# tensorlink-lab/tensorlink

Measured on NVIDIA H100. Metric: generate tokens/sec, higher is better.
Workload: dtype bf16

## Files before the change

include/tensorlink_b200.h:

```cpp
#ifndef TENSORLINK_B200_H
#define TENSORLINK_B200_H

#include <stddef.h>
#include <stdint.h>

#ifdef __cplusplus
extern "C" {
#endif

#define TL_ABI_VERSION 1

typedef enum {
    TL_OK = 0,
    TL_ERR_INVALID = -1,
    TL_ERR_CUDA = -2,
    TL_ERR_NO_DEVICE = -3,
    TL_ERR_WORKSPACE = -4
} tl_status;

#define TL_EPI_BIAS 1
#define TL_EPI_RESIDUAL 2
#define TL_EPI_SWIGLU 4
#define TL_EPI_OUT_F32 8
#define TL_EPI_ACCUM 16
#define TL_A_MN_MAJOR 32
#define TL_B_MN_MAJOR 64

int tl_abi_version(void);
const char* tl_last_error(void);
int tl_device_info(int* sm_count, int* cc_major, int* cc_minor);

int tl_rmsnorm_fwd(const void* x, const void* w, void* y, float* rstd_out, int rows, int H, float eps, void* stream);

int tl_embed_fwd(const int64_t* ids, const void* table, void* out, int n_tokens, int H, int vocab, void* stream);

int tl_gemm_bf16(const void* A, const void* B, void* C, int M, int N, int K, int lda, int ldb, int ldc,
                 const void* bias, const void* residual, int flags, void* stream);

size_t tl_gemm_splitk_ws(int M, int N);
int tl_gemm_bf16_ws(const void* A, const void* B, void* C, int M, int N, int K, int lda, int ldb, int ldc,
                    const void* bias, const void* residual, int flags, void* workspace, size_t ws_bytes, void* stream);
int tl_gemm_bf16_ws_norm(const void* A, const void* B, void* C, int M, int N, int K, int lda, int ldb, int ldc,
                         const void* bias, const void* residual, int flags, void* workspace, size_t ws_bytes,
                         const void* norm_w, float eps, void* H_out, void* stream);

int tl_gemv_bf16(const void* x, const void* W, void* y, int M, int N, int K, const void* bias,
                 const void* residual, const void* norm_w, float eps, int flags, void* stream);
int tl_gemv_bf16_pf(const void* x, const void* W, void* y, int M, int N, int K, const void* bias,
                    const void* residual, const void* norm_w, float eps, int flags, const void* next_W,
                    size_t next_bytes, void* stream);
#define TL_GEMV_COUNTER_WORDS 4
int tl_gemv_bf16_ctr(const void* x, const void* W, void* y, int M, int N, int K, const void* bias,
                     const void* residual, const void* norm_w, float eps, int flags, unsigned* counter,
                     const void* next_W, size_t next_bytes, void* stream);

#define TL_FP8_BLOCK 128
int tl_gemv_fp8(const void* x, const void* W, const float* scales, void* y, int M, int N, int K, const void* bias,
                const void* residual, const void* norm_w, float eps, int flags, void* stream);
int tl_gemv_fp8_ctr(const void* x, const void* W, const float* scales, void* y, int M, int N, int K, const void* bias,
                    const void* residual, const void* norm_w, float eps, int flags, unsigned* counter,
                    const void* next_W, size_t next_bytes, void* stream);
int tl_dequant_fp8(const void* W, const float* scales, void* out, int N, int K, void* stream);

int tl_rope_table(const float* inv_freq, void* cos_tab, void* sin_tab, int max_pos, int half_dim, void* stream);

int tl_rope_kv_fwd(const void* qkv, void* q_out, void* k_cache, void* v_cache, const int32_t* pos0_dev,
                   const void* cos_tab, const void* sin_tab, const void* q_norm_w, const void* k_norm_w,
                   float eps, int n_tokens, int S, int n_h, int n_kv, int d, int T_max, void* stream);

int tl_attn_prefill_fwd(const void* q, const void* k_cache, const void* v_cache, void* out, float* lse, int B,
// ... 182 lines not shown
```

tensorlink_b200/csrc/gemm.cu:

```cuda
#include <stdlib.h>

#include <mutex>
#include <unordered_map>

#include "gemm_common.cuh"

namespace tl {

constexpr int GEMM_THREADS = 384;

typedef CUresult (*EncodeTiledFn)(CUtensorMap*, CUtensorMapDataType, cuuint32_t, void*, const cuuint64_t*,
                                  const cuuint64_t*, const cuuint32_t*, const cuuint32_t*, CUtensorMapInterleave,
                                  CUtensorMapSwizzle, CUtensorMapL2promotion, CUtensorMapFloatOOBfill);

static EncodeTiledFn get_encode_fn() {
    static EncodeTiledFn fn = nullptr;
    static std::once_flag once;
    std::call_once(once, [] {
        void* p = nullptr;
        cudaDriverEntryPointQueryResult q;
        if (cudaGetDriverEntryPoint("cuTensorMapEncodeTiled", &p, cudaEnableDefault, &q) == cudaSuccess &&
            q == cudaDriverEntryPointSuccess)
            fn = (EncodeTiledFn)p;
        else
// ... 33 lines not shown
        if (it != cache.end()) {
            *out = it->second;
            return TL_OK;
        }
    }
    EncodeTiledFn enc = get_encode_fn();
    TL_REQUIRE(enc != nullptr, TL_ERR_CUDA, "cuTensorMapEncodeTiled not available from the driver");
    TL_REQUIRE(((uintptr_t)ptr & 15) == 0 && (ld * 2) % 16 == 0, TL_ERR_INVALID,
               "GEMM operand must be 16-byte aligned with a 16-byte-multiple row pitch (ptr=%p ld=%llu)", ptr,
               (unsigned long long)ld);
    cuuint64_t dims[2] = {inner, outer};
    cuuint64_t strides[1] = {ld * 2};
    cuuint32_t box[2] = {box_inner, box_outer};
    cuuint32_t estr[2] = {1, 1};
    CUresult r = enc(out, CU_TENSOR_MAP_DATA_TYPE_BFLOAT16, 2, const_cast<void*>(ptr), dims, strides, box, estr,
                     CU_TENSOR_MAP_INTERLEAVE_NONE, CU_TENSOR_MAP_SWIZZLE_128B, CU_TENSOR_MAP_L2_PROMOTION_L2_256B,
                     CU_TENSOR_MAP_FLOAT_OOB_FILL_NONE);
    TL_REQUIRE(r == CUDA_SUCCESS, TL_ERR_CUDA, "cuTensorMapEncodeTiled failed (%d) inner=%llu outer=%llu ld=%llu",
               (int)r, (unsigned long long)inner, (unsigned long long)outer, (unsigned long long)ld);
    std::lock_guard<std::mutex> g(mu);
    if (cache.size() > 4096) cache.clear();
    cache[key] = *out;
    return TL_OK;
}

template <int BN>
struct GemmCfg {
    static constexpr int A_BYTES = BM * BK * 2;
    static constexpr int B_BYTES = BN * BK * 2;
    static constexpr int STAGE_BYTES = A_BYTES + B_BYTES;
    static constexpr int STAGES = (BN == 128) ? 4 : 8;
    static constexpr int ACC_PITCH = BN + 4;
    static constexpr int ACC_BYTES = 64 * ACC_PITCH * 4;
    static constexpr int UNITS = BN >= 64 ? 2 * (BN / 64) : 2;
    static_assert(UNITS <= 4 && UNITS * EPI_STAGE_BYTES <= ACC_BYTES, "epilogue staging must fit in the accumulator tile");
    static constexpr int SMEM_BYTES = STAGES * STAGE_BYTES + 2 * ACC_BYTES + 1024  + 256 ;
};

__device__ __forceinline__ void named_bar_sync(int id, int threads) {
    asm volatile("bar.sync %0, %1;" ::"r"(id), "r"(threads) : "memory");
}

template <int BN, bool A_MN, bool B_MN>
__global__ void __launch_bounds__(GEMM_THREADS, 1)
gemm_bf16_kernel(const __grid_constant__ CUtensorMap tmA, const __grid_constant__ CUtensorMap tmB, void* __restrict__ Cv,
                 int M, int N, int K, int ldc, const bf16* __restrict__ bias, const bf16* __restrict__ residual,
                 int ldr, int flags, int k_splits, int kb_per) {
    using Cfg = GemmCfg<BN>;
    extern __shared__ unsigned char smem_dyn[];
    unsigned char* smem = reinterpret_cast<unsigned char*>((reinterpret_cast<uintptr_t>(smem_dyn) + 1023) & ~(uintptr_t)1023);
    float* acc_tile = reinterpret_cast<float*>(smem + Cfg::STAGES * Cfg::STAGE_BYTES);
    uint64_t* bars = reinterpret_cast<uint64_t*>(smem + Cfg::STAGES * Cfg::STAGE_BYTES + 2 * Cfg::ACC_BYTES);
    uint64_t* full_bar = bars;
    uint64_t* empty_bar = bars + Cfg::STAGES;

    const int wg = threadIdx.x >> 7, warp = threadIdx.x >> 5, lane = threadIdx.x & 31;
    const int tiles_m = (M + BM - 1) / BM, tiles_n = (N + BN - 1) / BN;
    const int mn_tiles = tiles_m * tiles_n;
    const int total_tiles = mn_tiles * k_splits;
    const int num_k = (K + BK - 1) / BK;

    if (threadIdx.x == 0) {
        tma_prefetch_desc(&tmA);
        tma_prefetch_desc(&tmB);
        for (int s = 0; s < Cfg::STAGES; ++s) {
            mbar_init(&full_bar[s], 1);
            mbar_init(&empty_bar[s], 8);
        }
        fence_barrier_init();
    }
    __syncthreads();

    if (wg == 0) {
// ... 48 lines not shown
            mbar_wait(&full_bar[stage], phase);
            {
                const uint32_t sa = smem_u32(smem + stage * Cfg::STAGE_BYTES) + (uint32_t)(cw * 8192);
                const uint32_t sb = smem_u32(smem + stage * Cfg::STAGE_BYTES + Cfg::A_BYTES);
                const uint64_t da = A_MN ? make_wgmma_desc_sw128(sa, 8192, 1024) : make_wgmma_desc_sw128(sa, 16, 1024);
                const uint64_t db = B_MN ? make_wgmma_desc_sw128(sb, 8192, 1024) : make_wgmma_desc_sw128(sb, 16, 1024);
                wgmma_fence_acc(d);
                wgmma_fence();
#pragma unroll
                for (int k = 0; k < BK / 16; ++k) {
                    const uint64_t ak = da + (uint64_t)((A_MN ? 2048 : 32) * k >> 4);
                    const uint64_t bk = db + (uint64_t)((B_MN ? 2048 : 32) * k >> 4);
                    const uint32_t acc = (kb > kb0 || k > 0) ? 1u : 0u;
                    if constexpr (BN == 128) wgmma_m64n128<A_MN ? 1 : 0, B_MN ? 1 : 0>(*reinterpret_cast<float(*)[64]>(d), ak, bk, acc);
                    else wgmma_m64n32<A_MN ? 1 : 0, B_MN ? 1 : 0>(*reinterpret_cast<float(*)[16]>(d), ak, bk, acc);
                }
                wgmma_commit();
                wgmma_fence_acc(d);
                wgmma_wait<1>();
            }
            if (prev >= 0) {
                __syncwarp();
                if (lane == 0) mbar_arrive(&empty_bar[prev]);
            }
            prev = stage;
            if (++stage == Cfg::STAGES) { stage = 0; phase ^= 1; }
        }
        wgmma_wait<0>();
        wgmma_fence_acc(d);
        __syncwarp();
        if (lane == 0) mbar_arrive(&empty_bar[prev]);
        if (!active) continue;

#pragma unroll
        for (int i = 0; i < BN / 2; i += 2) {
            const int r = 16 * wq + (lane >> 2) + 8 * ((i >> 1) & 1);
            const int c = 8 * (i >> 2) + 2 * (lane & 3);
            *reinterpret_cast<float2*>(my_acc + r * Cfg::ACC_PITCH + c) = make_float2(d[i], d[i + 1]);
        }
        named_bar_sync(1 + cw, 128);
        const int rh = wq & 1, ch = wq >> 1;
        const bool has_unit = wq < Cfg::UNITS;
        uint32_t r0[32], r1[32];
        if (has_unit) {
            const float* row = my_acc + (32 * rh + lane) * Cfg::ACC_PITCH + 64 * ch;
#pragma unroll
            for (int j = 0; j < 32; j += 4) {
                const float4 v = *reinterpret_cast<const float4*>(row + j);
                r0[j] = __float_as_uint(v.x); r0[j + 1] = __float_as_uint(v.y); r0[j + 2] = __float_as_uint(v.z); r0[j + 3] = __float_as_uint(v.w);
            }
#pragma unroll
            for (int j = 0; j < 32; j += 4) {
                float4 v = make_float4(0.f, 0.f, 0.f, 0.f);
                if (BN >= 64) v = *reinterpret_cast<const float4*>(row + 32 + j);
                r1[j] = __float_as_uint(v.x); r1[j + 1] = __float_as_uint(v.y); r1[j + 2] = __float_as_uint(v.z); r1[j + 3] = __float_as_uint(v.w);
            }
        }
        named_bar_sync(1 + cw, 128);
        if (has_unit) {
            void* Ct = k_splits > 1 ? (void*)(reinterpret_cast<float*>(Cv) + (size_t)ks * M * N) : Cv;
            unsigned char* stg = reinterpret_cast<unsigned char*>(my_acc) + wq * EPI_STAGE_BYTES;
            gemm_epilogue_chunk64(r0, r1, stg, Ct, m0 + 64 * cw + 32 * rh, lane, n0 + 64 * ch, M, N, ldc, bias, residual, ldr,
                                  flags, BN >= 64 ? 64 : BN);
        }
        named_bar_sync(1 + cw, 128);
    }
}

template <int BN, bool A_MN, bool B_MN>
static int launch_gemm(const void* A, const void* B, void* C, int M, int N, int K, int lda, int ldb, int ldc,
                       const void* bias, const void* residual, int flags, cudaStream_t st, int k_splits = 1, int kb_per = 0) {
    using Cfg = GemmCfg<BN>;
    CUtensorMap tmA, tmB;
    int rc;
    rc = A_MN ? make_tensor_map(&tmA, A, (uint64_t)M, (uint64_t)K, (uint64_t)lda, 64, BK)
              : make_tensor_map(&tmA, A, (uint64_t)K, (uint64_t)M, (uint64_t)lda, BK, BM);
    if (rc != TL_OK) return rc;
    rc = B_MN ? make_tensor_map(&tmB, B, (uint64_t)N, (uint64_t)K, (uint64_t)ldb, 64, BK)
              : make_tensor_map(&tmB, B, (uint64_t)K, (uint64_t)N, (uint64_t)ldb, BK, BN);
    if (rc != TL_OK) return rc;
    auto kern = gemm_bf16_kernel<BN, A_MN, B_MN>;
    static bool attr_done = false;
    if (!attr_done) {
        if (cudaFuncSetAttribute(kern, cudaFuncAttributeMaxDynamicSharedMemorySize, Cfg::SMEM_BYTES) != cudaSuccess)
            return check_launch("tl_gemm_bf16 (smem attr)");
        attr_done = true;
    }
    const int tiles = ((M + BM - 1) / BM) * ((N + BN - 1) / BN) * k_splits;
    const int grid = tiles < sm_count() ? tiles : sm_count();
    const int ldr = ldc;
    if (kb_per <= 0) kb_per = (K + BK - 1) / BK;
    kern<<<grid, GEMM_THREADS, Cfg::SMEM_BYTES, st>>>(tmA, tmB, C, M, N, K, ldc, (const bf16*)bias,
                                                      (const bf16*)residual, ldr, flags, k_splits, kb_per);
    return check_launch("tl_gemm_bf16");
}

template <int BN>
static int dispatch_major(bool a_mn, bool b_mn, const void* A, const void* B, void* C, int M, int N, int K, int lda,
                          int ldb, int ldc, const void* bias, const void* residual, int flags, cudaStream_t st) {
    if (!a_mn && !b_mn) return launch_gemm<BN, false, false>(A, B, C, M, N, K, lda, ldb, ldc, bias, residual, flags, st);
    if (!a_mn && b_mn) return launch_gemm<BN, false, true>(A, B, C, M, N, K, lda, ldb, ldc, bias, residual, flags, st);
    if (a_mn && !b_mn) return launch_gemm<BN, true, false>(A, B, C, M, N, K, lda, ldb, ldc, bias, residual, flags, st);
    return launch_gemm<BN, true, true>(A, B, C, M, N, K, lda, ldb, ldc, bias, residual, flags, st);
}

__global__ void splitk_reduce_kernel(const float* __restrict__ ws, void* __restrict__ Cv, int M, int N, int ldc, int splits,
                                     const bf16* __restrict__ bias, const bf16* __restrict__ residual, int ldr, int flags) {
    const int groups = N >> 3;
    const long long idx = (long long)blockIdx.x * blockDim.x + threadIdx.x;
    if (idx >= (long long)M * groups) return;
    const int m = (int)(idx / groups), c0 = (int)(idx - (long long)m * groups) * 8;
    float v[8];
#pragma unroll
    for (int j = 0; j < 8; ++j) v[j] = 0.f;
    for (int s = 0; s < splits; ++s) {
        const float4* p = reinterpret_cast<const float4*>(ws + ((size_t)s * M + m) * N + c0);
        const float4 a = p[0], b = p[1];
        v[0] += a.x; v[1] += a.y; v[2] += a.z; v[3] += a.w; v[4] += b.x; v[5] += b.y; v[6] += b.z; v[7] += b.w;
    }
    if (flags & TL_EPI_BIAS) {
#pragma unroll
        for (int j = 0; j < 8; ++j) v[j] += bf2f(bias[c0 + j]);
    }
    if (flags & TL_EPI_SWIGLU) {
        bf16* dst = reinterpret_cast<bf16*>(Cv) + (size_t)m * ldc + (c0 >> 1);
#pragma unroll
        for (int j = 0; j < 4; ++j) dst[j] = f2bf(rbf(silu_f(rbf(v[2 * j]))) * rbf(v[2 * j + 1]));
// ... 155 lines not shown
        if (splits > 8) splits = 8;
        int kb_per = (num_k + splits - 1) / splits;
        if (kb_per < 8) kb_per = 8;
        splits = (num_k + kb_per - 1) / kb_per;
        if (splits > 1 && ws_bytes >= (size_t)splits * M * N * sizeof(float)) {
            cudaStream_t st = (cudaStream_t)stream;
            int rc = launch_gemm<128, false, false>(A, B, workspace, M, N, K, lda, ldb, N, nullptr, nullptr, TL_EPI_OUT_F32, st,
                                                    splits, kb_per);
            if (rc != TL_OK) return rc;
            if (norm_w) {
                splitk_reduce_norm_kernel<<<M, RN_THREADS, 0, st>>>((const float*)workspace, (bf16*)C, M, N, ldc, splits,
                                                                    (const bf16*)bias, (const bf16*)residual, ldc, flags,
                                                                    (const bf16*)norm_w, eps, (bf16*)H_out);
                return check_launch("tl_gemm_bf16_ws_norm (reduce + norm)");
            }
            const long long items = (long long)M * (N >> 3);
            splitk_reduce_kernel<<<(unsigned)((items + 255) / 256), 256, 0, st>>>((const float*)workspace, C, M, N, ldc, splits,
                                                                                  (const bf16*)bias, (const bf16*)residual, ldc, flags);
            return check_launch("tl_gemm_bf16_ws (reduce)");
        }
    }
    int rc = tl_gemm_bf16(A, B, C, M, N, K, lda, ldb, ldc, bias, residual, flags, stream);
    if (rc != TL_OK || !norm_w) return rc;
    return tl_rmsnorm_fwd(C, norm_w, H_out, nullptr, M, N, eps, stream);
}

extern "C" int tl_gemm_bf16(const void* A, const void* B, void* C, int M, int N, int K, int lda, int ldb, int ldc,
                            const void* bias, const void* residual, int flags, void* stream) {
    using namespace tl;
    const int rc = check_gemm_args(M, N, K, lda, ldb, ldc, bias, residual, flags);
    if (rc != TL_OK) return rc;
    const bool a_mn = flags & TL_A_MN_MAJOR, b_mn = flags & TL_B_MN_MAJOR;
    cudaStream_t st = (cudaStream_t)stream;
    if (M <= BM && !b_mn && (long long)((N + 127) / 128) < 2LL * sm_count() && N % 32 == 0)
        return dispatch_major<32>(a_mn, b_mn, A, B, C, M, N, K, lda, ldb, ldc, bias, residual, flags, st);
    return dispatch_major<128>(a_mn, b_mn, A, B, C, M, N, K, lda, ldb, ldc, bias, residual, flags, st);
}
```

tensorlink_b200/ml/shard.py:

```python
from __future__ import annotations

from dataclasses import dataclass
from typing import Dict, List, Optional, Sequence

import torch

from .. import native as nat
from . import fp8 as F8
from .configs import ShardModelConfig, check_moe
from .weights import init_state_dict

ALIGN = 128


_GEMV_MAX_ROWS = None


def gemv_max_rows() -> int:
    global _GEMV_MAX_ROWS
    if _GEMV_MAX_ROWS is None:
        import os
        _GEMV_MAX_ROWS = max(1, min(8, int(os.environ.get("TL_GEMV_MAX_ROWS", "3"))))
    return _GEMV_MAX_ROWS


_FP8_GEMV_MAX_ROWS = None


def fp8_gemv_max_rows() -> int:
    global _FP8_GEMV_MAX_ROWS
    if _FP8_GEMV_MAX_ROWS is None:
        import os
        _FP8_GEMV_MAX_ROWS = max(1, min(8, int(os.environ.get("TL_FP8_GEMV_MAX_ROWS", "4"))))
    return _FP8_GEMV_MAX_ROWS


def fp8_gemv_rows(cfg: ShardModelConfig) -> int:
    K = max(cfg.hidden, cfg.q_dim, cfg.intermediate)
    fit = 0
    while fit < 4 and (fit + 1) * K * 2 + 256 * (fit + 1) <= 200 * 1024:
        fit += 1
    return min(fp8_gemv_max_rows(), fit)


def _rope_inv_freq(cfg: ShardModelConfig) -> torch.Tensor:
    d = cfg.head_dim
    return 1.0 / (cfg.rope_theta ** (torch.arange(0, d, 2, dtype=torch.int64).to(torch.float32) / d))


class ShardParams:

    def __init__(self, cfg: ShardModelConfig, layer_ids: Sequence[int], has_embed: bool, has_head: bool,
                 device, with_grad: bool = False, fp8: bool = False):
        if fp8 and with_grad:
            raise NotImplementedError("training with FP8 weights is not supported (load the model with training=False)")
        check_moe(cfg)
# ... 298 lines not shown
        cfg, dev, bf = self.cfg, self.device, torch.bfloat16
        return ShardBuffers(
            x=torch.empty(n, cfg.hidden, dtype=bf, device=dev), h=torch.empty(n, cfg.hidden, dtype=bf, device=dev),
            qkv=torch.empty(n, cfg.qkv_dim, dtype=bf, device=dev), q=torch.empty(n, cfg.q_dim, dtype=bf, device=dev),
            attn=torch.empty(n, cfg.q_dim, dtype=bf, device=dev),
            act=torch.empty(n, cfg.intermediate, dtype=bf, device=dev))

    def _alloc_bufs(self, n: int):
        self.bufs = self._make_bufs(n)
        self.n_alloc = n

    def _dbufs(self, n: int) -> ShardBuffers:
        b = self.dbufs
        return ShardBuffers(b.x[:n], b.h[:n], b.qkv[:n], b.q[:n], b.attn[:n], b.act[:n], b.moe)

    def _bufs(self, n: int) -> ShardBuffers:
        if n > self.n_alloc:
            self._alloc_bufs(n)
        b = self.bufs
        if self.cfg.is_moe and (self.moe_pf is None or self.moe_pf.n < n):
            self.moe_pf = MoeBuffers(self.cfg, n, self.device)
        return ShardBuffers(b.x[:n], b.h[:n], b.qkv[:n], b.q[:n], b.attn[:n], b.act[:n], self.moe_pf)

    def reset_cache(self, past_len: int = 0):
        self.pos_dev.fill_(past_len)
        self.kvlen_dev.fill_(past_len)

    def _gemv(self, x: torch.Tensor, name: str, **kw) -> torch.Tensor:
        p = self.p
        if p.fp8:
            return nat.gemv_fp8(x, p.v[name], p.s[name], **kw)
        return nat.gemv(x, p.v[name], **kw)

    def _gemm(self, a: torch.Tensor, name: str, **kw) -> torch.Tensor:
        p = self.p
        w = nat.dequant_fp8(p.v[name], p.s[name], out=p.deq) if p.fp8 else p.v[name]
        return nat.gemm(a, w, **kw)

    def gemv_rows(self) -> int:
        return fp8_gemv_rows(self.cfg) if self.p.fp8 else gemv_max_rows()

    def _kv_start(self):
        return self.kv_start_dev if self.ragged else None

    def _layer_prefill(self, j: int, x: torch.Tensor, B: int, S: int, past_len: int, w: ShardBuffers):
        cfg, v, li = self.cfg, self.p.v, self.layer_ids[j]
        ks = self._kv_start()
        nat.rmsnorm_fwd(x, v[f"l{li}.ln1"], cfg.rms_eps, out=w.h)
        self._gemm(w.h, f"l{li}.wqkv", out=w.qkv, bias=v.get(f"l{li}.bqkv"))
        nat.rope_kv_fwd(w.qkv, w.q, self.kc[j], self.vc[j], self.pos_dev, self.cos, self.sin, v.get(f"l{li}.qn"),
                        v.get(f"l{li}.kn"), cfg.rms_eps, S, cfg.n_heads, cfg.n_kv_heads, cfg.head_dim, kv_start=ks)
        nat.attn_prefill_fwd(w.q, self.kc[j], self.vc[j], w.attn, None, B, S, past_len, cfg.n_heads, cfg.n_kv_heads,
                             cfg.head_dim, self.scale, kv_start=ks)
        self._gemm(w.attn, f"l{li}.wo", out=x, residual=x)
        nat.rmsnorm_fwd(x, v[f"l{li}.ln2"], cfg.rms_eps, out=w.h)
        if cfg.is_moe:
            self._moe_grouped(li, x, w.h, w.moe)
            return
        self._gemm(w.h, f"l{li}.wgu", out=w.act, flags=nat.EPI_SWIGLU)
        self._gemm(w.act, f"l{li}.wd", out=x, residual=x)

    def _moe_grouped(self, li: int, x: torch.Tensor, h: torch.Tensor, mb: MoeBuffers, out: Optional[torch.Tensor] = None):
        cfg, v = self.cfg, self.p.v
        n, k = h.shape[0], cfg.top_k
        T = nat.moe_max_tiles(n, cfg.n_experts, k)
        nat.gemm(h, v[f"l{li}.router"], out=mb.logits[:n])
        row_of, tiles = mb.row_of[:n * k], mb.tiles[:T]
        nat.moe_route(mb.logits[:n], k, cfg.norm_topk_prob, mb.ids[:n], mb.wts[:n], (mb.counts, mb.offsets, row_of, tiles))
        nat.moe_gather(h, row_of, mb.hg[:T * 128], k)
        nat.moe_gemm(mb.hg[:T * 128], v[f"l{li}.ewgu"], mb.act[:T * 128], tiles, flags=nat.EPI_SWIGLU)
        nat.moe_gemm(mb.act[:T * 128], v[f"l{li}.ewd"], mb.y[:T * 128], tiles)
        nat.moe_combine(mb.y[:T * 128], row_of, mb.wts[:n], x, x if out is None else out)

    def _layer_decode_moe(self, j: int, x: torch.Tensor, B: int, w: ShardBuffers, out: Optional[torch.Tensor], attention):
        cfg, v, li, mb = self.cfg, self.p.v, self.layer_ids[j], w.moe
        ctr = self.gemv_ctr[j]
        self._gemv(x, f"l{li}.wqkv", out=w.qkv, bias=v.get(f"l{li}.bqkv"), norm_w=v[f"l{li}.ln1"], eps=cfg.rms_eps,
                   next_w=v[f"l{li}.wo"], counter=ctr[0])
        attention(j, li, B, w)
        self._gemv(w.attn, f"l{li}.wo", out=x, residual=x, next_w=v[f"l{li}.router"], counter=ctr[1])
        nat.rmsnorm_fwd(x, v[f"l{li}.ln2"], cfg.rms_eps, out=w.h)
        nat.gemv(w.h, v[f"l{li}.router"], out=mb.logits[:B], counter=ctr[2])
        nat.moe_route(mb.logits[:B], cfg.top_k, cfg.norm_topk_prob, mb.ids[:B], mb.wts[:B])
        act = mb.act[:B * cfg.top_k]
        nat.moe_gemv(w.h, v[f"l{li}.ewgu"], act, mb.ids[:B], flags=nat.EPI_SWIGLU)
        nat.moe_gemv(act, v[f"l{li}.ewd"], x if out is None else out, mb.ids[:B], wts=mb.wts[:B], residual=x,
                     flags=nat.EPI_RESIDUAL)

    FUSED_DECODE_MAX_T = 2048

    def _decode_attention(self, j: int, li: int, B: int, w: ShardBuffers):
        cfg, v = self.cfg, self.p.v
        ks = self._kv_start()
# ... 245 lines not shown
```

tensorlink_b200/native.py:

```python
from __future__ import annotations

import ctypes
import os
from ctypes import POINTER, c_char_p, c_float, c_int, c_int32, c_size_t, c_void_p
from typing import Optional

import torch

_HERE = os.path.dirname(os.path.abspath(__file__))
LIB_PATH = os.path.join(_HERE, "csrc", "libtensorlink_b200.so")

EPI_BIAS, EPI_RESIDUAL, EPI_SWIGLU, EPI_OUT_F32, EPI_ACCUM, A_MN_MAJOR, B_MN_MAJOR = 1, 2, 4, 8, 16, 32, 64


class NativeError(RuntimeError):
    pass


_LOG_ARGS = [c_void_p, c_void_p, c_void_p, c_int, c_int, c_int, c_void_p]
_WARP_ARGS = [c_float, c_float, c_float, c_float]

_SIGS = {
    "tl_abi_version": (c_int, []),
    "tl_last_error": (c_char_p, []),
    "tl_device_info": (c_int, [POINTER(c_int), POINTER(c_int), POINTER(c_int)]),
    "tl_rmsnorm_fwd": (c_int, [c_void_p, c_void_p, c_void_p, c_void_p, c_int, c_int, c_float, c_void_p]),
    "tl_embed_fwd": (c_int, [c_void_p, c_void_p, c_void_p, c_int, c_int, c_int, c_void_p]),
    "tl_gemm_bf16": (c_int, [c_void_p, c_void_p, c_void_p, c_int, c_int, c_int, c_int, c_int, c_int,
                             c_void_p, c_void_p, c_int, c_void_p]),
    "tl_gemm_splitk_ws": (c_size_t, [c_int, c_int]),
    "tl_gemm_bf16_ws": (c_int, [c_void_p, c_void_p, c_void_p, c_int, c_int, c_int, c_int, c_int, c_int,
                                c_void_p, c_void_p, c_int, c_void_p, c_size_t, c_void_p]),
    "tl_gemm_bf16_ws_norm": (c_int, [c_void_p, c_void_p, c_void_p, c_int, c_int, c_int, c_int, c_int, c_int,
                                     c_void_p, c_void_p, c_int, c_void_p, c_size_t, c_void_p, c_float, c_void_p, c_void_p]),
    "tl_gemv_bf16": (c_int, [c_void_p, c_void_p, c_void_p, c_int, c_int, c_int, c_void_p, c_void_p, c_void_p,
                             c_float, c_int, c_void_p]),
    "tl_gemv_bf16_pf": (c_int, [c_void_p, c_void_p, c_void_p, c_int, c_int, c_int, c_void_p, c_void_p, c_void_p,
                                c_float, c_int, c_void_p, c_size_t, c_void_p]),
    "tl_gemv_bf16_ctr": (c_int, [c_void_p, c_void_p, c_void_p, c_int, c_int, c_int, c_void_p, c_void_p, c_void_p,
                                 c_float, c_int, c_void_p, c_void_p, c_size_t, c_void_p]),
    "tl_gemv_fp8": (c_int, [c_void_p, c_void_p, c_void_p, c_void_p, c_int, c_int, c_int, c_void_p, c_void_p, c_void_p,
                            c_float, c_int, c_void_p]),
    "tl_gemv_fp8_ctr": (c_int, [c_void_p, c_void_p, c_void_p, c_void_p, c_int, c_int, c_int, c_void_p, c_void_p,
                                c_void_p, c_float, c_int, c_void_p, c_void_p, c_size_t, c_void_p]),
    "tl_dequant_fp8": (c_int, [c_void_p, c_void_p, c_void_p, c_int, c_int, c_void_p]),
    "tl_rope_table": (c_int, [c_void_p, c_void_p, c_void_p, c_int, c_int, c_void_p]),
    "tl_rope_kv_fwd": (c_int, [c_void_p, c_void_p, c_void_p, c_void_p, c_void_p, c_void_p, c_void_p, c_void_p,
                               c_void_p, c_float, c_int, c_int, c_int, c_int, c_int, c_int, c_void_p]),
    "tl_attn_prefill_fwd": (c_int, [c_void_p, c_void_p, c_void_p, c_void_p, c_void_p, c_int, c_int, c_int, c_int,
                                    c_int, c_int, c_int, c_float, c_void_p]),
    "tl_attn_decode_ws": (c_size_t, [c_int, c_int, c_int, c_int]),
    "tl_attn_decode_fwd": (c_int, [c_void_p, c_void_p, c_void_p, c_void_p, c_void_p, c_void_p, c_size_t, c_int,
                                   c_int, c_int, c_int, c_int, c_float, c_void_p]),
    "tl_attn_decode_fused": (c_int, [c_void_p] * 9 + [c_float, c_int, c_int, c_int, c_int, c_int, c_float, c_void_p]),
    "tl_attn_verify_ws": (c_size_t, [c_int, c_int, c_int, c_int]),
    "tl_attn_verify_fwd": (c_int, [c_void_p] * 6 + [c_size_t, c_int, c_int, c_int, c_int, c_int, c_float, c_void_p]),
    "tl_prompt_lookup_draft": (c_int, [c_void_p, c_void_p, c_int, c_void_p, c_int, c_void_p, c_void_p, c_void_p]),
    "tl_prompt_lookup_accept": (c_int, [c_void_p] * 6 + [c_int, c_int, c_void_p, c_void_p, c_void_p, c_int, c_void_p,
                                                         c_void_p, c_int, c_void_p]),
    "tl_assist_prep": (c_int, [c_void_p, c_void_p, c_int] + [c_void_p] * 5),
    "tl_rope_kv_fwd_rows": (c_int, [c_void_p, c_void_p, c_void_p, c_void_p, c_void_p, c_void_p, c_void_p, c_void_p,
                                    c_void_p, c_float, c_int, c_int, c_int, c_int, c_int, c_int, c_void_p, c_void_p]),
# ... 184 lines not shown
         h_out: Optional[torch.Tensor] = None) -> torch.Tensor:
    require_device()
    _bf16(a, b, bias, residual)
    a_mn, b_mn = bool(flags & A_MN_MAJOR), bool(flags & B_MN_MAJOR)
    if M is None:
        M = a.shape[1] if a_mn else a.shape[0]
    if K is None:
        K = a.shape[0] if a_mn else a.shape[1]
    if N is None:
        N = b.shape[1] if b_mn else b.shape[0]
    c_cols = N // 2 if flags & EPI_SWIGLU else N
    if out is None:
        out = torch.empty(M, c_cols, dtype=torch.float32 if flags & EPI_OUT_F32 else torch.bfloat16, device=a.device)
    if bias is not None:
        flags |= EPI_BIAS
    if residual is not None:
        flags |= EPI_RESIDUAL
    if norm_w is not None:
        assert h_out is not None and h_out.dtype == torch.bfloat16 and h_out.is_contiguous() and h_out.shape == out.shape
        _check(load().tl_gemm_bf16_ws_norm(_p(a), _p(b), _p(out), M, N, K, a.stride(0), b.stride(0), out.stride(0), _p(bias),
                                           _p(residual), flags, _p(ws), 0 if ws is None else ws.numel() * ws.element_size(),
                                           _p(norm_w), eps, _p(h_out), _stream()), "tl_gemm_bf16_ws_norm")
        return out
    if ws is not None:
        _check(load().tl_gemm_bf16_ws(_p(a), _p(b), _p(out), M, N, K, a.stride(0), b.stride(0), out.stride(0), _p(bias),
                                      _p(residual), flags, _p(ws), ws.numel() * ws.element_size(), _stream()),
               "tl_gemm_bf16_ws")
        return out
    _check(load().tl_gemm_bf16(_p(a), _p(b), _p(out), M, N, K, a.stride(0), b.stride(0), out.stride(0), _p(bias),
                               _p(residual), flags, _stream()), "tl_gemm_bf16")
    return out


_PREFETCH_BYTES = None


def prefetch_bytes() -> int:
    global _PREFETCH_BYTES
    if _PREFETCH_BYTES is None:
        _PREFETCH_BYTES = int(float(os.environ.get("TL_PREFETCH_MB", "8")) * (1 << 20))
    return _PREFETCH_BYTES


def gemv_counters(*shape, device=None) -> torch.Tensor:
    return torch.zeros(*shape, GEMV_COUNTER_WORDS, dtype=torch.int32, device=device)


def gemv(x: torch.Tensor, w: torch.Tensor, out: Optional[torch.Tensor] = None, *, bias=None, residual=None,
         norm_w=None, eps: float = 1e-6, flags: int = 0, next_w: Optional[torch.Tensor] = None,
         counter: Optional[torch.Tensor] = None) -> torch.Tensor:
    require_device()
    _bf16(x, w, bias, residual, norm_w, out)
    M, K = x.shape
    N = w.shape[0]
    if out is None:
        out = torch.empty(M, N // 2 if flags & EPI_SWIGLU else N, dtype=torch.bfloat16, device=x.device)
    if bias is not None:
        flags |= EPI_BIAS
    if residual is not None:
        flags |= EPI_RESIDUAL
    nb = min(next_w.numel() * next_w.element_size(), prefetch_bytes()) if next_w is not None else 0
    _check(load().tl_gemv_bf16_ctr(_p(x), _p(w), _p(out), M, N, K, _p(bias), _p(residual), _p(norm_w), eps, flags,
                                   _p(counter), _p(next_w) if nb else None, nb, _stream()), "tl_gemv_bf16_ctr")
    return out


# ... 591 lines not shown
```

Before: 201.0.

## Add weight-streaming GEMM kernel for small-M prefill with deep TMA pipeline

Adds a new persistent GEMM kernel for M<=64 that keeps the shared A block resident and streams weight tiles through as many TMA stages as fit in shared memory, splitting N units across SMs and pairing two N-tiles per pass when M is small. Prefill layers with at most 64 rows now use it by default, aiming to turn small-batch prefill GEMMs into bandwidth-bound weight streaming with less tile overhead. The epilogue is factored into a shared helper that can process wide tiles in 64-column chunks. Risks include occupancy and load imbalance across SMs and correctness constraints (K-major only, bf16 output).

```diff
diff --git a/include/tensorlink_b200.h b/include/tensorlink_b200.h
--- a/include/tensorlink_b200.h
+++ b/include/tensorlink_b200.h
@@ -36,6 +36,9 @@
 
 int tl_gemm_bf16(const void* A, const void* B, void* C, int M, int N, int K, int lda, int ldb, int ldc,
                  const void* bias, const void* residual, int flags, void* stream);
+
+int tl_gemm_stream_bf16(const void* A, const void* B, void* C, int M, int N, int K, int lda, int ldb, int ldc,
+                        const void* bias, const void* residual, int flags, void* stream);
 
 size_t tl_gemm_splitk_ws(int M, int N);
 int tl_gemm_bf16_ws(const void* A, const void* B, void* C, int M, int N, int K, int lda, int ldb, int ldc,
diff --git a/tensorlink_b200/csrc/gemm.cu b/tensorlink_b200/csrc/gemm.cu
--- a/tensorlink_b200/csrc/gemm.cu
+++ b/tensorlink_b200/csrc/gemm.cu
@@ -89,13 +89,55 @@
     static constexpr int STAGES = (BN == 128) ? 4 : 8;
     static constexpr int ACC_PITCH = BN + 4;
     static constexpr int ACC_BYTES = 64 * ACC_PITCH * 4;
-    static constexpr int UNITS = BN >= 64 ? 2 * (BN / 64) : 2;
-    static_assert(UNITS <= 4 && UNITS * EPI_STAGE_BYTES <= ACC_BYTES, "epilogue staging must fit in the accumulator tile");
     static constexpr int SMEM_BYTES = STAGES * STAGE_BYTES + 2 * ACC_BYTES + 1024  + 256 ;
 };
 
 __device__ __forceinline__ void named_bar_sync(int id, int threads) {
     asm volatile("bar.sync %0, %1;" ::"r"(id), "r"(threads) : "memory");
+}
+
+template <int BN, int TC = BN>
+__device__ __forceinline__ void tile_epilogue(const float (&d)[BN / 2], float* my_acc, int wq, int lane, int cw, void* Ct,
+                                              int row0, int n0, int M, int N, int ldc,
+                                              const bf16* __restrict__ bias, const bf16* __restrict__ residual, int ldr,
+                                              int flags) {
+    constexpr int PITCH = TC + 4;
+    constexpr int UNITS = TC >= 64 ? 2 * (TC / 64) : 2;
+    static_assert(BN % TC == 0 && UNITS <= 4 && UNITS * EPI_STAGE_BYTES <= 64 * PITCH * 4, "epilogue staging must fit in the tile");
+#pragma unroll
+    for (int h = 0; h < BN / TC; ++h) {
+#pragma unroll
+        for (int i = h * (TC / 2); i < (h + 1) * (TC / 2); i += 2) {
+            const int r = 16 * wq + (lane >> 2) + 8 * ((i >> 1) & 1);
+            const int c = 8 * (i >> 2) + 2 * (lane & 3) - h * TC;
+            *reinterpret_cast<float2*>(my_acc + r * PITCH + c) = make_float2(d[i], d[i + 1]);
+        }
+        named_bar_sync(1 + cw, 128);
+        const int rh = wq & 1, ch = wq >> 1;
+        const bool has_unit = wq < UNITS;
+        uint32_t r0[32], r1[32];
+        if (has_unit) {
+            const float* row = my_acc + (32 * rh + lane) * PITCH + 64 * ch;
+#pragma unroll
+            for (int j = 0; j < 32; j += 4) {
+                const float4 v = *reinterpret_cast<const float4*>(row + j);
+                r0[j] = __float_as_uint(v.x); r0[j + 1] = __float_as_uint(v.y); r0[j + 2] = __float_as_uint(v.z); r0[j + 3] = __float_as_uint(v.w);
+            }
+#pragma unroll
+            for (int j = 0; j < 32; j += 4) {
+                float4 v = make_float4(0.f, 0.f, 0.f, 0.f);
+                if (TC >= 64) v = *reinterpret_cast<const float4*>(row + 32 + j);
+                r1[j] = __float_as_uint(v.x); r1[j + 1] = __float_as_uint(v.y); r1[j + 2] = __float_as_uint(v.z); r1[j + 3] = __float_as_uint(v.w);
+            }
+        }
+        named_bar_sync(1 + cw, 128);
+        if (has_unit) {
+            unsigned char* stg = reinterpret_cast<unsigned char*>(my_acc) + wq * EPI_STAGE_BYTES;
+            gemm_epilogue_chunk64(r0, r1, stg, Ct, row0 + 32 * rh, lane, n0 + h * TC + 64 * ch, M, N, ldc, bias, residual, ldr,
+                                  flags, TC >= 64 ? 64 : TC);
+        }
+        named_bar_sync(1 + cw, 128);
+    }
 }
 
 template <int BN, bool A_MN, bool B_MN>
@@ -210,38 +252,8 @@
         if (lane == 0) mbar_arrive(&empty_bar[prev]);
         if (!active) continue;
 
-#pragma unroll
-        for (int i = 0; i < BN / 2; i += 2) {
-            const int r = 16 * wq + (lane >> 2) + 8 * ((i >> 1) & 1);
-            const int c = 8 * (i >> 2) + 2 * (lane & 3);
-            *reinterpret_cast<float2*>(my_acc + r * Cfg::ACC_PITCH + c) = make_float2(d[i], d[i + 1]);
-        }
-        named_bar_sync(1 + cw, 128);
-        const int rh = wq & 1, ch = wq >> 1;
-        const bool has_unit = wq < Cfg::UNITS;
-        uint32_t r0[32], r1[32];
-        if (has_unit) {
-            const float* row = my_acc + (32 * rh + lane) * Cfg::ACC_PITCH + 64 * ch;
-#pragma unroll
-            for (int j = 0; j < 32; j += 4) {
-                const float4 v = *reinterpret_cast<const float4*>(row + j);
-                r0[j] = __float_as_uint(v.x); r0[j + 1] = __float_as_uint(v.y); r0[j + 2] = __float_as_uint(v.z); r0[j + 3] = __float_as_uint(v.w);
-            }
-#pragma unroll
-            for (int j = 0; j < 32; j += 4) {
-                float4 v = make_float4(0.f, 0.f, 0.f, 0.f);
-                if (BN >= 64) v = *reinterpret_cast<const float4*>(row + 32 + j);
-                r1[j] = __float_as_uint(v.x); r1[j + 1] = __float_as_uint(v.y); r1[j + 2] = __float_as_uint(v.z); r1[j + 3] = __float_as_uint(v.w);
-            }
-        }
-        named_bar_sync(1 + cw, 128);
-        if (has_unit) {
-            void* Ct = k_splits > 1 ? (void*)(reinterpret_cast<float*>(Cv) + (size_t)ks * M * N) : Cv;
-            unsigned char* stg = reinterpret_cast<unsigned char*>(my_acc) + wq * EPI_STAGE_BYTES;
-            gemm_epilogue_chunk64(r0, r1, stg, Ct, m0 + 64 * cw + 32 * rh, lane, n0 + 64 * ch, M, N, ldc, bias, residual, ldr,
-                                  flags, BN >= 64 ? 64 : BN);
-        }
-        named_bar_sync(1 + cw, 128);
+        void* Ct = k_splits > 1 ? (void*)(reinterpret_cast<float*>(Cv) + (size_t)ks * M * N) : Cv;
+        tile_epilogue<BN>(d, my_acc, wq, lane, cw, Ct, m0 + 64 * cw, n0, M, N, ldc, bias, residual, ldr, flags);
     }
 }
 
@@ -271,6 +283,170 @@
     kern<<<grid, GEMM_THREADS, Cfg::SMEM_BYTES, st>>>(tmA, tmB, C, M, N, K, ldc, (const bf16*)bias,
                                                       (const bf16*)residual, ldr, flags, k_splits, kb_per);
     return check_launch("tl_gemm_bf16");
+}
+
+constexpr int STREAM_MAX_STAGES = 32;
+constexpr int STREAM_SMEM_LIMIT = 227 * 1024;
+
+template <int BN>
+struct StreamCfg {
+    static constexpr int B_BYTES = BN * BK * 2;
+    static constexpr int TC = BN > 64 ? 64 : BN;
+    static constexpr int ACC_PITCH = TC + 4;
+    static constexpr int ACC_BYTES = 64 * ACC_PITCH * 4;
+    static constexpr int FIXED_BYTES = 2 * ACC_BYTES + 1024  + 2 * STREAM_MAX_STAGES * 8 ;
+};
+
+template <int BN>
+__global__ void __launch_bounds__(GEMM_THREADS, 1)
+gemm_stream_bf16_kernel(const __grid_constant__ CUtensorMap tmA, const __grid_constant__ CUtensorMap tmB, void* __restrict__ Cv,
+                        int M, int N, int K, int ldc, const bf16* __restrict__ bias, const bf16* __restrict__ residual,
+                        int flags, int units, int upc, int pair, int stages, int a_bytes, int a_rows) {
+    using Cfg = StreamCfg<BN>;
+    constexpr int B_BYTES = Cfg::B_BYTES;
+    extern __shared__ unsigned char smem_dyn[];
+    unsigned char* smem = reinterpret_cast<unsigned char*>((reinterpret_cast<uintptr_t>(smem_dyn) + 1023) & ~(uintptr_t)1023);
+    const int stage_bytes = a_bytes + (pair ? 2 : 1) * B_BYTES;
+    float* acc_tile = reinterpret_cast<float*>(smem + stages * stage_bytes);
+    uint64_t* full_bar = reinterpret_cast<uint64_t*>(smem + stages * stage_bytes + 2 * Cfg::ACC_BYTES);
+    uint64_t* empty_bar = full_bar + STREAM_MAX_STAGES;
+
+    const int wg = threadIdx.x >> 7, warp = threadIdx.x >> 5, lane = threadIdx.x & 31;
+    const int num_k = (K + BK - 1) / BK;
+    const int u_begin = blockIdx.x * upc, u_end = min(units, u_begin + upc);
+    const int per_pass = pair ? 2 : 1;
+
+    if (threadIdx.x == 0) {
+        tma_prefetch_desc(&tmA);
+        tma_prefetch_desc(&tmB);
+        for (int s = 0; s < stages; ++s) {
+            mbar_init(&full_bar[s], 1);
+            mbar_init(&empty_bar[s], 8);
+        }
+        fence_barrier_init();
+    }
+    const int pad_vecs = (a_bytes - a_rows * BK * 2) / 16;
+    for (int i = threadIdx.x; i < stages * pad_vecs; i += GEMM_THREADS) {
+        const int st = i / pad_vecs;
+        *reinterpret_cast<uint4*>(smem + st * stage_bytes + a_rows * BK * 2 + (i - st * pad_vecs) * 16) = make_uint4(0, 0, 0, 0);
+    }
+    asm volatile("fence.proxy.async.shared::cta;\n" ::: "memory");
+    __syncthreads();
+
+    if (wg == 0) {
+        asm volatile("setmaxnreg.dec.sync.aligned.u32 40;\n" ::: "memory");
+        if (threadIdx.x == 0) {
+            int stage = 0;
+            uint32_t phase = 0;
+            for (int u = u_begin; u < u_end; u += per_pass) {
+                const int nb = min(per_pass, u_end - u);
+                for (int kb = 0; kb < num_k; ++kb) {
+                    mbar_wait(&empty_bar[stage], phase ^ 1);
+                    unsigned char* sa = smem + stage * stage_bytes;
+                    mbar_expect_tx(&full_bar[stage], a_rows * BK * 2 + nb * B_BYTES);
+                    tma_load_2d(sa, &tmA, &full_bar[stage], kb * BK, 0);
+                    for (int j = 0; j < nb; ++j)
+                        tma_load_2d(sa + a_bytes + j * B_BYTES, &tmB, &full_bar[stage], kb * BK, (u + j) * BN);
+                    if (++stage == stages) { stage = 0; phase ^= 1; }
+                }
+            }
+        }
+        return;
+    }
+
+    asm volatile("setmaxnreg.inc.sync.aligned.u32 232;\n" ::: "memory");
+    const int cw = wg - 1;
+    const int wq = warp & 3;
+    float* my_acc = acc_tile + cw * 64 * Cfg::ACC_PITCH;
+    int stage = 0;
+    uint32_t phase = 0;
+    for (int u = u_begin; u < u_end; u += per_pass) {
+        const bool has_job = pair ? (u + cw < u_end) : (64 * cw < M);
+        const uint32_t a_off = pair ? 0u : (uint32_t)(cw * 8192);
+        const uint32_t b_off = (uint32_t)(a_bytes + (pair ? cw * B_BYTES : 0));
+        float d[BN / 2];
+#pragma unroll
+        for (int i = 0; i < BN / 2; ++i) d[i] = 0.f;
+        int prev = -1;
+        for (int kb = 0; kb < num_k; ++kb) {
+            mbar_wait(&full_bar[stage], phase);
+            if (has_job) {
+                const uint32_t base = smem_u32(smem + stage * stage_bytes);
+                const uint64_t da = make_wgmma_desc_sw128(base + a_off, 16, 1024);
+                const uint64_t db = make_wgmma_desc_sw128(base + b_off, 16, 1024);
+                wgmma_fence_acc(d);
+                wgmma_fence();
+#pragma unroll
+                for (int k = 0; k < BK / 16; ++k) {
+                    const uint64_t ak = da + (uint64_t)(32 * k >> 4);
+                    const uint64_t bk = db + (uint64_t)(32 * k >> 4);
+                    const uint32_t acc = (kb > 0 || k > 0) ? 1u : 0u;
+                    if constexpr (BN == 128) wgmma_m64n128<0, 0>(*reinterpret_cast<float(*)[64]>(d), ak, bk, acc);
+                    else wgmma_m64n32<0, 0>(*reinterpret_cast<float(*)[16]>(d), ak, bk, acc);
+                }
+                wgmma_commit();
+                wgmma_fence_acc(d);
+                wgmma_wait<1>();
+            }
+            if (prev >= 0) {
+                __syncwarp();
+                if (lane == 0) mbar_arrive(&empty_bar[prev]);
+            }
+            prev = stage;
+            if (++stage == stages) { stage = 0; phase ^= 1; }
+        }
+        wgmma_wait<0>();
+        wgmma_fence_acc(d);
+        __syncwarp();
+        if (lane == 0) mbar_arrive(&empty_bar[prev]);
+        if (!has_job) continue;
+        tile_epilogue<BN, Cfg::TC>(d, my_acc, wq, lane, cw, Cv, pair ? 0 : 64 * cw, (pair ? u + cw : u) * BN, M, N, ldc, bias,
+                          residual, ldc, flags);
+    }
+}
+
+struct StreamPlan {
+    int units, upc, grid, pair, a_bytes, a_rows, stages, smem;
+};
+template <int BN>
+static StreamPlan stream_plan(int M, int N) {
+    StreamPlan p;
+    p.units = (N + BN - 1) / BN;
+    p.upc = (p.units + sm_count() - 1) / sm_count();
+    p.grid = (p.units + p.upc - 1) / p.upc;
+    p.pair = M <= 64 && p.upc >= 2;
+    p.a_bytes = (M <= 64 ? 64 : 128) * BK * 2;
+    p.a_rows = (M + 7) / 8 * 8;
+    const int stage_bytes = p.a_bytes + (p.pair ? 2 : 1) * StreamCfg<BN>::B_BYTES;
+    p.stages = (STREAM_SMEM_LIMIT - StreamCfg<BN>::FIXED_BYTES) / stage_bytes;
+    if (p.stages > STREAM_MAX_STAGES) p.stages = STREAM_MAX_STAGES;
+    p.smem = p.stages * stage_bytes + StreamCfg<BN>::FIXED_BYTES;
+    return p;
+}
+
+template <int BN>
+static int launch_gemm_stream(const void* A, const void* B, void* C, int M, int N, int K, int lda, int ldb, int ldc,
+                              const void* bias, const void* residual, int flags, cudaStream_t st) {
+    const StreamPlan p = stream_plan<BN>(M, N);
+    CUtensorMap tmA, tmB;
+    int rc = make_tensor_map(&tmA, A, (uint64_t)K, (uint64_t)M, (uint64_t)lda, BK, (uint32_t)p.a_rows);
+    if (rc != TL_OK) return rc;
+    rc = make_tensor_map(&tmB, B, (uint64_t)K, (uint64_t)N, (uint64_t)ldb, BK, BN);
+    if (rc != TL_OK) return rc;
+    auto kern = gemm_stream_bf16_kernel<BN>;
+    static bool attr_done = false;
+    if (!attr_done) {
+        if (cudaFuncSetAttribute(kern, cudaFuncAttributeMaxDynamicSharedMemorySize, STREAM_SMEM_LIMIT) != cudaSuccess)
+            return check_launch("tl_gemm_stream_bf16 (smem attr)");
+        attr_done = true;
+    }
+    kern<<<p.grid, GEMM_THREADS, p.smem, st>>>(tmA, tmB, C, M, N, K, ldc, (const bf16*)bias, (const bf16*)residual, flags,
+                                               p.units, p.upc, p.pair, p.stages, p.a_bytes, p.a_rows);
+    return check_launch("tl_gemm_stream_bf16");
+}
+
+static int gemm_tile_n(int M, int N, bool b_mn) {
+    return (M <= BM && !b_mn && (long long)((N + 127) / 128) < 2LL * sm_count() && N % 32 == 0) ? 32 : 128;
 }
 
 template <int BN>
@@ -492,7 +668,25 @@
     if (rc != TL_OK) return rc;
     const bool a_mn = flags & TL_A_MN_MAJOR, b_mn = flags & TL_B_MN_MAJOR;
     cudaStream_t st = (cudaStream_t)stream;
-    if (M <= BM && !b_mn && (long long)((N + 127) / 128) < 2LL * sm_count() && N % 32 == 0)
+    if (gemm_tile_n(M, N, b_mn) == 32)
         return dispatch_major<32>(a_mn, b_mn, A, B, C, M, N, K, lda, ldb, ldc, bias, residual, flags, st);
     return dispatch_major<128>(a_mn, b_mn, A, B, C, M, N, K, lda, ldb, ldc, bias, residual, flags, st);
 }
+
+extern "C" int tl_gemm_stream_bf16(const void* A, const void* B, void* C, int M, int N, int K, int lda, int ldb, int ldc,
+                                   const void* bias, const void* residual, int flags, void* stream) {
+    using namespace tl;
+    const int rc = check_gemm_args(M, N, K, lda, ldb, ldc, bias, residual, flags);
+    if (rc != TL_OK) return rc;
+    TL_REQUIRE(M <= BM, TL_ERR_INVALID, "tl_gemm_stream_bf16: M must be <= %d (M=%d)", BM, M);
+    TL_REQUIRE(!(flags & (TL_A_MN_MAJOR | TL_B_MN_MAJOR)), TL_ERR_INVALID, "tl_gemm_stream_bf16: A and B must be K-major");
+    TL_REQUIRE(!(flags & (TL_EPI_OUT_F32 | TL_EPI_ACCUM)), TL_ERR_INVALID, "tl_gemm_stream_bf16: bf16 output only (no OUT_F32 / ACCUM)");
+    TL_REQUIRE(N % 32 == 0, TL_ERR_INVALID, "tl_gemm_stream_bf16: N must be a multiple of 32 (N=%d)", N);
+    TL_REQUIRE(lda % 8 == 0 && ldb % 8 == 0 && ((uintptr_t)C & 15) == 0 && ((uintptr_t)bias & 15) == 0 &&
+                   ((uintptr_t)residual & 15) == 0, TL_ERR_INVALID,
+               "tl_gemm_stream_bf16: lda/ldb must be multiples of 8 and C / bias / residual 16-byte aligned");
+    cudaStream_t st = (cudaStream_t)stream;
+    if (gemm_tile_n(M, N, false) == 32)
+        return launch_gemm_stream<32>(A, B, C, M, N, K, lda, ldb, ldc, bias, residual, flags, st);
+    return launch_gemm_stream<128>(A, B, C, M, N, K, lda, ldb, ldc, bias, residual, flags, st);
+}
diff --git a/tensorlink_b200/ml/shard.py b/tensorlink_b200/ml/shard.py
--- a/tensorlink_b200/ml/shard.py
+++ b/tensorlink_b200/ml/shard.py
@@ -22,6 +22,11 @@
         import os
         _GEMV_MAX_ROWS = max(1, min(8, int(os.environ.get("TL_GEMV_MAX_ROWS", "3"))))
     return _GEMV_MAX_ROWS
+
+
+def prefill_gemm_stream(rows: int) -> bool:
+    import os
+    return rows <= 64 and os.environ.get("TL_PREFILL_GEMM", "stream") != "tiled"
 
 
 _FP8_GEMV_MAX_ROWS = None
@@ -386,10 +391,10 @@
             return nat.gemv_fp8(x, p.v[name], p.s[name], **kw)
         return nat.gemv(x, p.v[name], **kw)
 
-    def _gemm(self, a: torch.Tensor, name: str, **kw) -> torch.Tensor:
+    def _gemm(self, a: torch.Tensor, name: str, stream: bool = False, **kw) -> torch.Tensor:
         p = self.p
         w = nat.dequant_fp8(p.v[name], p.s[name], out=p.deq) if p.fp8 else p.v[name]
-        return nat.gemm(a, w, **kw)
+        return nat.gemm_stream(a, w, **kw) if stream else nat.gemm(a, w, **kw)
 
     def gemv_rows(self) -> int:
         return fp8_gemv_rows(self.cfg) if self.p.fp8 else gemv_max_rows()
@@ -400,19 +405,20 @@
     def _layer_prefill(self, j: int, x: torch.Tensor, B: int, S: int, past_len: int, w: ShardBuffers):
         cfg, v, li = self.cfg, self.p.v, self.layer_ids[j]
         ks = self._kv_start()
+        st = prefill_gemm_stream(B * S)
         nat.rmsnorm_fwd(x, v[f"l{li}.ln1"], cfg.rms_eps, out=w.h)
-        self._gemm(w.h, f"l{li}.wqkv", out=w.qkv, bias=v.get(f"l{li}.bqkv"))
+        self._gemm(w.h, f"l{li}.wqkv", st, out=w.qkv, bias=v.get(f"l{li}.bqkv"))
         nat.rope_kv_fwd(w.qkv, w.q, self.kc[j], self.vc[j], self.pos_dev, self.cos, self.sin, v.get(f"l{li}.qn"),
                         v.get(f"l{li}.kn"), cfg.rms_eps, S, cfg.n_heads, cfg.n_kv_heads, cfg.head_dim, kv_start=ks)
         nat.attn_prefill_fwd(w.q, self.kc[j], self.vc[j], w.attn, None, B, S, past_len, cfg.n_heads, cfg.n_kv_heads,
                              cfg.head_dim, self.scale, kv_start=ks)
-        self._gemm(w.attn, f"l{li}.wo", out=x, residual=x)
+        self._gemm(w.attn, f"l{li}.wo", st, out=x, residual=x)
         nat.rmsnorm_fwd(x, v[f"l{li}.ln2"], cfg.rms_eps, out=w.h)
         if cfg.is_moe:
             self._moe_grouped(li, x, w.h, w.moe)
             return
-        self._gemm(w.h, f"l{li}.wgu", out=w.act, flags=nat.EPI_SWIGLU)
-        self._gemm(w.act, f"l{li}.wd", out=x, residual=x)
+        self._gemm(w.h, f"l{li}.wgu", st, out=w.act, flags=nat.EPI_SWIGLU)
+        self._gemm(w.act, f"l{li}.wd", st, out=x, residual=x)
 
     def _moe_grouped(self, li: int, x: torch.Tensor, h: torch.Tensor, mb: MoeBuffers, out: Optional[torch.Tensor] = None):
         cfg, v = self.cfg, self.p.v
diff --git a/tensorlink_b200/native.py b/tensorlink_b200/native.py
--- a/tensorlink_b200/native.py
+++ b/tensorlink_b200/native.py
@@ -28,6 +28,8 @@
     "tl_embed_fwd": (c_int, [c_void_p, c_void_p, c_void_p, c_int, c_int, c_int, c_void_p]),
     "tl_gemm_bf16": (c_int, [c_void_p, c_void_p, c_void_p, c_int, c_int, c_int, c_int, c_int, c_int,
                              c_void_p, c_void_p, c_int, c_void_p]),
+    "tl_gemm_stream_bf16": (c_int, [c_void_p, c_void_p, c_void_p, c_int, c_int, c_int, c_int, c_int, c_int,
+                                    c_void_p, c_void_p, c_int, c_void_p]),
     "tl_gemm_splitk_ws": (c_size_t, [c_int, c_int]),
     "tl_gemm_bf16_ws": (c_int, [c_void_p, c_void_p, c_void_p, c_int, c_int, c_int, c_int, c_int, c_int,
                                 c_void_p, c_void_p, c_int, c_void_p, c_size_t, c_void_p]),
@@ -278,6 +280,22 @@
     return out
 
 
+def gemm_stream(a: torch.Tensor, b: torch.Tensor, out: Optional[torch.Tensor] = None, *, bias=None, residual=None,
+                flags: int = 0) -> torch.Tensor:
+    require_device()
+    _bf16(a, b, bias, residual)
+    M, K, N = a.shape[0], a.shape[1], b.shape[0]
+    if out is None:
+        out = torch.empty(M, N // 2 if flags & EPI_SWIGLU else N, dtype=torch.bfloat16, device=a.device)
+    if bias is not None:
+        flags |= EPI_BIAS
+    if residual is not None:
+        flags |= EPI_RESIDUAL
+    _check(load().tl_gemm_stream_bf16(_p(a), _p(b), _p(out), M, N, K, a.stride(0), b.stride(0), out.stride(0), _p(bias),
+                                      _p(residual), flags, _stream()), "tl_gemm_stream_bf16")
+    return out
+
+
 _PREFETCH_BYTES = None
 
 
```

New measurement: 201.7, median of 6. No clear change (+0.3%).
